# a1q123456/image_stitching

Measured on AMD Instinct MI355X. Metric: 4K frames stitched/sec, higher is better.
Workload: dtype u8

## Files before the change

host/job.cpp:

```cpp
#include "job.hpp"
#include <cstring>

namespace mis {

StitchJob::StitchJob(int device, int width, int height, const std::vector<CameraParams>& cameras, const StitchConfig& cfg)
    : JobCore("mis::StitchJob", "", device, nullptr, width, height, cameras, cfg) {}

StitchJob::~StitchJob() {
    mis_image_free(cctx_, &pano_);
    mis_image_free(cctx_, &mask_);
}

void StitchJob::finalize() {
    if (pano_.data && (pano_.width != key_.pano.width || pano_.height != key_.pano.height)) { mis_image_free(cctx_, &pano_); mis_image_free(cctx_, &mask_); pano_ = MisImage{}; mask_ = MisImage{}; }
    if (!pano_.data) { pano_ = MisImage{}; mask_ = MisImage{}; pano_.mem = mask_.mem = MIS_MEM_DEVICE; }
    check(cctx_, mis_blender_blend(blender_, &pano_, &mask_), "mis_blender_blend");
}

JobOutput StitchJob::run(const std::vector<MisImage>& frames) {
    if ((int)frames.size() != n_) throw std::runtime_error("StitchJob::run: one frame per camera");
    JobOutput out;
    check(cctx_, mis_context_wait(cctx_, ctx_), "mis_context_wait");
    const MisImage* work = work_frames(frames);
    prep_.arm([this] { if (spec_ok_) prepare(everyone_); });
    check(ctx_, mis_orb_on_enqueued(orb_, &Hook::fire, &prep_), "mis_orb_on_enqueued");
    std::vector<MisFeatures> feats(n_);
    std::memset(feats.data(), 0, sizeof(MisFeatures) * n_);
    const int rc_f = mis_orb_detect_batch(orb_, work, n_, feats.data());
    mis_orb_on_enqueued(orb_, nullptr, nullptr);
    check(ctx_, rc_f, "mis_orb_detect_batch");
    prep_.finish();
    for (int i = 0; i < n_; i++) { feats[i].img_idx = i; out.num_features.push_back(feats[i].n); }
    const MisMatchParams mp = reset_matches();
    match_.arm([this, &frames] {
        if (!spec_ok_) return;
        fence_knn();
        compose(frames, everyone_, everyone_);
        finalize();
    });
    check(ctx_, mis_match_on_enqueued(ctx_, &Hook::fire, &match_), "mis_match_on_enqueued");
    const int rc = mis_match_all_pairs(ctx_, feats.data(), n_, &mp, pairwise_.data());
    mis_match_on_enqueued(ctx_, nullptr, nullptr);
    for (auto& f : feats) mis_features_free(ctx_, &f);
    check(ctx_, rc, "mis_match_all_pairs");
    match_.finish();
// ... 23 lines not shown
```

image_stitching_amd/_capi.py:

```python
import ctypes as C
import os
import re

_HERE = os.path.dirname(os.path.abspath(__file__))
LIB_PATH = os.path.join(_HERE, "libmistitch.so")
HEADER_PATH = os.path.join(os.path.dirname(_HERE), "include", "mistitch.h")

MIS_OK = 0
MIS_FENCE_TIMEOUT = 1
MEM_HOST, MEM_DEVICE = 0, 1
U8, S16, F32 = 0, 1, 2
INTER_NEAREST, INTER_LINEAR = 0, 1
BORDER_CONSTANT, BORDER_REFLECT = 0, 2
BLEND_NO, BLEND_FEATHER, BLEND_MULTI_BAND = 0, 1, 2
WARP_SPHERICAL, WARP_CYLINDRICAL, WARP_PLANE = 0, 1, 2


class MisPoint(C.Structure):
    _fields_ = [("x", C.c_int), ("y", C.c_int)]


class MisSize(C.Structure):
    _fields_ = [("width", C.c_int), ("height", C.c_int)]

# ... 59 lines not shown
PROTOTYPES = {
    "mis_context_create": (_i, [_i, _vp, _P(_vp)]),
    "mis_stream_create": (_i, [_i, _i, _P(_vp)]),
    "mis_stream_destroy": (_i, [_vp]),
    "mis_context_destroy": (_i, [_vp]),
    "mis_context_synchronize": (_i, [_vp]),
    "mis_context_wait": (_i, [_vp, _vp]),
    "mis_last_error": (C.c_char_p, [_vp]),
    "mis_version": (C.c_char_p, []),
    "mis_image_free": (_i, [_vp, _P(MisImage)]),
    "mis_orb_default_params": (None, [_P(MisOrbParams)]),
    "mis_orb_create": (_i, [_vp, _P(MisOrbParams), _i, _i, _P(_vp)]),
    "mis_orb_destroy": (_i, [_vp]),
    "mis_orb_detect": (_i, [_vp, _P(MisImage), _P(MisFeatures)]),
    "mis_orb_detect_batch": (_i, [_vp, _P(MisImage), _i, _P(MisFeatures)]),
    "mis_orb_on_enqueued": (_i, [_vp, _vp, _vp]),
    "mis_features_download": (_i, [_vp, _P(MisFeatures), _vp, _vp]),
    "mis_features_upload": (_i, [_vp, _i, _i, _i, _vp, _vp, _i, _i, _P(MisFeatures)]),
    "mis_features_free": (_i, [_vp, _P(MisFeatures)]),
    "mis_orb_debug_level": (_i, [_vp, _i, _i, _vp, _P(_i), _P(_i)]),
    "mis_sift_default_params": (None, [_P(MisSiftParams)]),
    "mis_sift_create": (_i, [_vp, _P(MisSiftParams), _i, _i, _P(_vp)]),
    "mis_sift_destroy": (_i, [_vp]),
    "mis_sift_detect": (_i, [_vp, _P(MisImage), _P(MisFeatures)]),
    "mis_sift_detect_batch": (_i, [_vp, _P(MisImage), _i, _P(MisFeatures)]),
    "mis_sift_debug_level": (_i, [_vp, _P(MisImage), _i, _i, _i, _vp, _P(_i), _P(_i)]),
    "mis_match_default_params": (None, [_P(MisMatchParams)]),
    "mis_match_all_pairs": (_i, [_vp, _P(MisFeatures), _i, _P(MisMatchParams), _P(MisMatchesInfo)]),
    "mis_match_pairs_sharded": (_i, [_vp, _P(MisFeatures), _i, _P(MisMatchParams), _i, _i, _P(MisMatchesInfo)]),
    "mis_matches_free": (_i, [_P(MisMatchesInfo), _i]),
# ... 81 lines not shown
```

image_stitching_amd/csrc/common.h:

```cpp
#pragma once
#include <hip/hip_runtime.h>
#include <stdint.h>
#include <stdio.h>
#include <string.h>
#include <string>
#include <vector>
#include "../../include/mistitch.h"

struct MisWorkspace {
    virtual ~MisWorkspace() {}
};

struct MisContext {
    int device = 0;
    int num_cu = 256;
    MisWorkspace* match_ws = nullptr;
    MisWorkspace* resize_ws = nullptr;
    std::vector<std::pair<size_t, void*>> pool;
    hipStream_t stream = nullptr;
    bool own_stream = false;
    std::string err;
    void* stage = nullptr;
    size_t stage_bytes = 0;
    hipStream_t aux[2] = {nullptr, nullptr};
    void* roi_pinned = nullptr;
    size_t roi_pinned_bytes = 0;
    void* host_stage = nullptr;
    size_t host_stage_bytes = 0;
};

int mis_set_error(MisContext* ctx, int code, const char* fmt, ...);
int mis_host_stage(MisContext* ctx, size_t bytes, void** out);
int mis_dev_stage(MisContext* ctx, size_t bytes, void** out);
int mis_pool_alloc(MisContext* ctx, size_t bytes, void** out, size_t* got, MisContext* errs = nullptr);
int mis_aux_stream(MisContext* ctx, int k, hipStream_t* out);
void mis_pool_free(MisContext* ctx, void* p, size_t bytes);
int mis_feat_block_alloc(MisContext* ctx, size_t bytes, void** out, MisContext* errs = nullptr);

#define MIS_HIP(ctx, call)                                                                             \
    do {                                                                                               \
        hipError_t e_ = (call);                                                                        \
// ... 39 lines not shown
```

image_stitching_amd/csrc/context.hip:

```cpp
#include "common.h"
#include <mutex>
#include <stdarg.h>

int mis_set_error(MisContext* ctx, int code, const char* fmt, ...) {
    char buf[512];
    va_list ap;
    va_start(ap, fmt);
    vsnprintf(buf, sizeof(buf), fmt, ap);
    va_end(ap);
    if (ctx) ctx->err = buf;
    return code;
}

static std::mutex g_pool_mutex;
int mis_pool_alloc(MisContext* ctx, size_t bytes, void** out, size_t* got, MisContext* errs) {
    std::lock_guard<std::mutex> lock(g_pool_mutex);
    int best = -1;
    for (int i = 0; i < (int)ctx->pool.size(); i++)
        if (ctx->pool[i].first >= bytes && ctx->pool[i].first <= 2 * bytes && (best < 0 || ctx->pool[i].first < ctx->pool[best].first)) best = i;
    if (best >= 0) {
        *out = ctx->pool[best].second; *got = ctx->pool[best].first;
        ctx->pool.erase(ctx->pool.begin() + best);
        return MIS_OK;
    }
// ... 52 lines not shown
    ctx->stream = (hipStream_t)stream;
    *out = ctx;
    return MIS_OK;
}

extern "C" int mis_context_destroy(MisContext* ctx) {
    if (!ctx) return MIS_OK;
    hipSetDevice(ctx->device);
    hipStreamSynchronize(ctx->stream);
    delete ctx->match_ws;
    delete ctx->resize_ws;
    for (auto& b : ctx->pool) hipFree(b.second);
    if (ctx->stage) hipFree(ctx->stage);
    if (ctx->roi_pinned) hipHostFree(ctx->roi_pinned);
    if (ctx->host_stage) hipHostFree(ctx->host_stage);
    for (hipStream_t& a : ctx->aux) if (a) { hipStreamSynchronize(a); hipStreamDestroy(a); a = nullptr; }
    if (ctx->own_stream) hipStreamDestroy(ctx->stream);
    delete ctx;
    return MIS_OK;
}

extern "C" int mis_stream_create(int device, int priority, void** out) {
    if (!out) return MIS_E_INVALID;
    *out = nullptr;
    if (hipSetDevice(device) != hipSuccess) return MIS_E_HIP;
    int least = 0, greatest = 0;
    if (hipDeviceGetStreamPriorityRange(&least, &greatest) != hipSuccess) return MIS_E_HIP;
    const int pr = priority > 0 ? least : (priority < 0 ? greatest : 0);
    hipStream_t s = nullptr;
    if (hipStreamCreateWithPriority(&s, hipStreamNonBlocking, pr) != hipSuccess) return MIS_E_HIP;
// ... 137 lines not shown
```

image_stitching_amd/csrc/match.hip:

```cpp
#include "common.h"
#include <thread>
#include <chrono>
#include <atomic>
#include "dev_math.h"
#include "homography.h"
#include <algorithm>
#include <vector>

namespace {

struct FeatDev {
    const uint8_t* desc;
    const MisKeyPoint* kps;
    int n, w, h;
};

struct PairDesc {
    int i, j;
    size_t knn_off12, knn_off21;
    size_t m_off;
    int cap;
};

constexpr int KNN_TILE = 256;
// ... 546 lines not shown

void invert3(const double* H, double* I) {
    double d = H[0] * (H[4] * H[8] - H[5] * H[7]) - H[1] * (H[3] * H[8] - H[5] * H[6]) + H[2] * (H[3] * H[7] - H[4] * H[6]);
    if (d != 0.) d = 1. / d;
    I[0] = (H[4] * H[8] - H[5] * H[7]) * d; I[1] = (H[2] * H[7] - H[1] * H[8]) * d; I[2] = (H[1] * H[5] - H[2] * H[4]) * d;
    I[3] = (H[5] * H[6] - H[3] * H[8]) * d; I[4] = (H[0] * H[8] - H[2] * H[6]) * d; I[5] = (H[2] * H[3] - H[0] * H[5]) * d;
    I[6] = (H[3] * H[7] - H[4] * H[6]) * d; I[7] = (H[1] * H[6] - H[0] * H[7]) * d; I[8] = (H[0] * H[4] - H[1] * H[3]) * d;
}

struct Arena {
    void* p = nullptr;
    size_t bytes = 0;
    bool host = false;
    hipError_t reserve(size_t need) {
        if (need <= bytes) return hipSuccess;
        if (p) { hipError_t e = host ? hipHostFree(p) : hipFree(p); p = nullptr; bytes = 0; if (e != hipSuccess) return e; }
        need = need + need / 4 + 4096;
        hipError_t e = host ? hipHostMalloc(&p, need, hipHostMallocDefault) : hipMalloc(&p, need);
        if (e == hipSuccess) bytes = need;
        return e;
    }
    void release() { if (p) { if (host) hipHostFree(p); else hipFree(p); } p = nullptr; bytes = 0; }
};

struct MatchWorkspace : MisWorkspace {
    Arena dev, pinned, l2;
    HomoBatch b1, b2, b3;
    hipStream_t side = nullptr, third = nullptr;
    OwnedEvent ev_phase0, ev_side_done, ev_phase1, ev_third_done, ev_matches;
    OwnedEvent ev_knn;
    OwnedEvent ev_draw1;
    OwnedEvent tev[8];
    hipEvent_t ev_gate = nullptr;
    std::atomic<long long> seq{0}, knn_seq{0};
    OwnedEvent ev_lists;
    void (*enqueued_cb)(void*) = nullptr;
    void* enqueued_user = nullptr;
    MatchWorkspace() { pinned.host = true; }
    ~MatchWorkspace() override {
        dev.release(); pinned.release(); l2.release();
        homo_batch_release(&b1); homo_batch_release(&b2); homo_batch_release(&b3);
    }
    hipError_t events_ready() {
        for (OwnedEvent* e : {&ev_knn, &ev_matches, &ev_lists, &ev_phase0, &ev_draw1, &ev_side_done, &ev_phase1, &ev_third_done})
            if (const hipError_t r = e->ready()) return r;
        return hipSuccess;
    }
};

MatchWorkspace* workspace(MisContext* ctx) {
    if (!ctx->match_ws) ctx->match_ws = new MatchWorkspace();
    return static_cast<MatchWorkspace*>(ctx->match_ws);
}

struct Carver {
    uintptr_t base = 0;
    size_t off = 0;
    size_t take(size_t bytes) { size_t o = off; off += mis_align_up(bytes ? bytes : 1, 256); return o; }
    void* at(size_t bytes) { return (void*)(base + take(bytes)); }
// ... 283 lines not shown
    MIS_HIP(ctx, hipSetDevice(ctx->device));
    const auto t_begin = std::chrono::steady_clock::now();
    struct SeqGuard {
        MatchWorkspace* ws; long long seq;
        ~SeqGuard() { if (ws->knn_seq.load() < seq) ws->knn_seq.store(seq); }
    } seq_guard{workspace(ctx), 0};
    seq_guard.seq = ++seq_guard.ws->seq;
    for (int i = 0; i < n * n; i++) init_info(&out[i]);
    MatchPlan pl;
    int rc;
    if ((rc = plan_match(ctx, feats, n, rank, world, &pl)) != MIS_OK) return rc;
    const int np = (int)pl.pairs.size();
    if (np == 0) return MIS_OK;
    MatchWorkspace* ws = workspace(ctx);
    hipStream_t st = ctx->stream;
    MIS_HIP(ctx, hipStreamSynchronize(st));
    MatchDev d; MatchPinned h;
    if ((rc = carve_dev(ctx, ws->dev, pl, &d)) != MIS_OK) return rc;
    for (HomoBatch* b : {&ws->b1, &ws->b2, &ws->b3})
        if ((rc = homo_batch_reserve(ctx, b, np, (long long)pl.m_total, p->max_iters)) != MIS_OK) return rc;
    if ((rc = carve_pinned(ctx, ws->pinned, pl, &h)) != MIS_OK) return rc;
    memcpy(h.feats, pl.fd.data(), sizeof(FeatDev) * n);
    memcpy(h.pairs, pl.pairs.data(), sizeof(PairDesc) * np);
    MIS_HIP(ctx, hipMemcpyAsync(d.feats, h.feats, sizeof(FeatDev) * n, hipMemcpyHostToDevice, st));
    MIS_HIP(ctx, hipMemcpyAsync(d.pairs, h.pairs, sizeof(PairDesc) * np, hipMemcpyHostToDevice, st));
    *h.l2_bad = 0;
    if ((rc = enqueue_knn(ctx, ws, pl, feats, d, h)) != MIS_OK) return rc;
    MIS_HIP(ctx, ws->events_ready());
    MIS_HIP(ctx, hipEventRecord(ws->ev_knn.ev, st));
    ws->ev_gate = ws->ev_knn.ev;
    hipLaunchKernelGGL(ratio_union_kernel, dim3(np), dim3(1024), 0, st, (const FeatDev*)d.feats, (const PairDesc*)d.pairs, (const int*)d.idx,
                       (const float*)d.dist, 1.f - p->match_conf, d.matches, d.src, d.dst, d.nm);
    hipLaunchKernelGGL(first_calls_kernel, dim3((np + 127) / 128), dim3(128), 0, st, (const PairDesc*)d.pairs, np, (const int*)d.nm, (const float*)d.src,
                       (const float*)d.dst, d.mask, p->num_matches_thresh1, ws->b1.calls, d.out);
    if ((rc = enqueue_chains(ctx, ws, np, p, d, h)) != MIS_OK) {
        if (ws->side) hipStreamSynchronize(ws->side);
        if (ws->third) hipStreamSynchronize(ws->third);
        hipStreamSynchronize(st);
        return rc;
    }
    MIS_HIP(ctx, hipGetLastError());
    enqueue_results(ws, np, pl.m_total, d, h, st);
    ws->knn_seq.store(seq_guard.seq);
    if (ws->enqueued_cb) {
        void (*cb)(void*) = ws->enqueued_cb;
        void* user = ws->enqueued_user;
        ws->enqueued_cb = nullptr; ws->enqueued_user = nullptr;
        cb(user);
        MIS_HIP(ctx, hipSetDevice(ctx->device));
    }
    const auto tq = std::chrono::steady_clock::now();
    std::chrono::steady_clock::time_point ts;
    if ((rc = assemble_matches(ctx, ws, pl, h, n, out, &ts)) != MIS_OK) return rc;
    if (match_trace()) trace_report(ws, t_begin, tq, ts);
    return MIS_OK;
}

// ... 165 lines not shown
```

image_stitching_amd/csrc/orb.hip:

```cpp
#include "common.h"
#include "dev_math.h"
#include <algorithm>
#include <cmath>
#include <mutex>
#include <unordered_map>

#define ORB_MAX_LEVELS 16
#define ORB_BORDER 32

namespace {

struct LevelDesc {
    int w, h;
    int pp;
    int sp;
    size_t pad_off;
    size_t map_off;
    float scale;
    int nfeat;
    int n2;
    int tiles_x, tiles_y, tile_off;
    int cap1, cand_off;
    int cap2, fin_off;
    int tab_off;
// ... 849 lines not shown
#ifndef DD_UNROLL
#define DD_UNROLL 1
#endif
#pragma unroll DD_UNROLL
    for (int bit = 0; bit < 4; bit++) {
        float x0 = (float)pat[4 * bit], y0 = (float)pat[4 * bit + 1], x1 = (float)pat[4 * bit + 2], y1 = (float)pat[4 * bit + 3];
        int ix0 = mis_round_f(x0 * ca - y0 * sa), iy0 = mis_round_f(x0 * sa + y0 * ca);
        int ix1 = mis_round_f(x1 * ca - y1 * sa), iy1 = mis_round_f(x1 * sa + y1 * ca);
        const int t0 = blurred(ix0, iy0), t1 = blurred(ix1, iy1);
        val |= (t0 < t1) << (bit + 4 * h);
    }
    val |= __shfl_xor(val, 32);
    if (h == 0) desc[(size_t)i * 32 + b] = (uint8_t)val;
}

constexpr int ORB_GATHER_MAX = 96;
struct GatherPtrs { const int* p[ORB_GATHER_MAX]; };
__global__ void gather_ints_kernel(GatherPtrs g, int n, int* __restrict__ out) {
    const int i = blockIdx.x * blockDim.x + threadIdx.x;
    if (i < n) out[i] = *g.p[i];
}

}

struct MisOrb {
    MisContext* ctx = nullptr;
    void (*enqueued_cb)(void*) = nullptr;
    void* enqueued_user = nullptr;
    MisOrbParams p;
    int max_w = 0, max_h = 0;
    int cur_w = 0, cur_h = 0;
    Levels L;
    Work w;
    size_t ws_stride = 0;
    int ws_frames = 0;
    int umax_host[64] = {0};
    int8_t pattern_host[1024] = {0};
    void* mem = nullptr;
    size_t pad_bytes = 0, map_bytes = 0;
    int cand_total = 0, fin_total = 0, tab_total = 0, surv_total = 0, out_cap = 0;
    std::vector<int> tab_host;
    int* host_counts = nullptr;
    bool direct_describe = false;
};

namespace {

void linear_exact_coeffs(int dlen, int slen, int* ofs, int* m1) {
    double inv = (double)dlen / (double)slen, scale = 1.0 / inv;
    for (int i = 0; i < dlen; i++) {
        double v = ((double)i + 0.5) * scale - 0.5;
        int iv = (int)floor(v);
        if (iv < 0) { ofs[i] = 0; m1[i] = 0; }
        else if (iv >= slen - 1) { ofs[i] = slen - 1; m1[i] = 0; }
        else { ofs[i] = iv; m1[i] = (int)lrint((v - (double)iv) * 256.0); }
    }
}
// ... 84 lines not shown
    std::lock_guard<std::mutex> lock(g_feat_mutex);
    g_feat_sizes[mem] = got;
    return MIS_OK;
}

inline uint32_t* feat_lxy(const MisFeatures* f, int cap) {
    size_t kb = mis_align_up(sizeof(MisKeyPoint) * (size_t)cap, 256), db = mis_align_up((size_t)cap * f->desc_cols * mis_dtype_size(f->desc_dtype), 256);
    return (uint32_t*)((uint8_t*)f->owner_ + kb + db);
}
inline int* feat_count(const MisFeatures* f, int cap) {
    size_t kb = mis_align_up(sizeof(MisKeyPoint) * (size_t)cap, 256), db = mis_align_up((size_t)cap * f->desc_cols * mis_dtype_size(f->desc_dtype), 256);
    size_t lb = mis_align_up(sizeof(uint32_t) * (size_t)cap, 256);
    return (int*)((uint8_t*)f->owner_ + kb + db + lb);
}

int enqueue_detect_group(MisOrb* o, const DevView* img, int w, int h, MisFeatures* out, int ng) {
    MisContext* ctx = o->ctx;
    const Levels& L = o->L;
    const Work& W = o->w;
    hipStream_t st = ctx->stream;
    const LevelDesc& d0 = L.d[0];
    const size_t ws = o->ws_stride;
    const unsigned nf = (unsigned)ng;
    OrbIO io;
    for (int k = 0; k < ORB_BATCH; k++) {
        const int q = k < ng ? k : 0;
        io.src[k] = (const uint8_t*)img[q].data; io.sstride[k] = img[q].stride;
        io.aligned[k] = (img[q].stride % 4 == 0) && ((uintptr_t)img[q].data % 4 == 0);
        io.kps[k] = out[q].keypoints; io.lxy[k] = feat_lxy(&out[q], o->out_cap); io.n_dev[k] = feat_count(&out[q], o->out_cap);
        io.desc[k] = (uint8_t*)out[q].descriptors;
    }
// ... 6 lines not shown
                           d.h, d.pp, W.tab + d.tab_off, ws);
    }
    const int pw0 = d0.w + 2 * ORB_BORDER, ph0 = d0.h + 2 * ORB_BORDER;
    hipLaunchKernelGGL((border_kernel<true>), dim3((d0.h * 16 + 255) / 256, 1, L.n * nf), dim3(256), 0, st, L, W.pad, ws);
    hipLaunchKernelGGL((border_kernel<false>), dim3((pw0 + 1023) / 1024, 2 * ORB_BORDER / 4, L.n * nf), dim3(256), 0, st, L, W.pad, ws);
    dim3 gmap((d0.w + FT_COLS - 1) / FT_COLS, (d0.h + FT_ROWS - 1) / FT_ROWS, L.n * nf);
    hipLaunchKernelGGL(fast_nms_kernel, gmap, dim3(256), 0, st, L, W.pad, W.hist, W.tile_cnt, W.surv_xy, W.surv_sc, ws);
    hipLaunchKernelGGL(fast_cut_kernel, dim3(L.n, nf), dim3(256), 0, st, L, W.hist, W.thr, W.flags, ws);
    hipLaunchKernelGGL(compact_kernel, dim3((d0.tiles_x * d0.tiles_y + CT_TILES - 1) / CT_TILES, L.n, nf), dim3(256), 0, st, L, W.tile_cnt, W.surv_xy, W.surv_sc, W.thr, W.cnt1,
                       W.cand_xy, W.cand_resp, ws);
    const int use_harris = o->p.score_type == 0;
    if (use_harris)
        hipLaunchKernelGGL(harris_kernel, dim3((L.d[0].cap1 + 255) / 256, L.n, nf), dim3(256), 0, st, L, W.pad, W.cnt1, W.cand_xy, W.cand_resp, ws);
    hipLaunchKernelGGL(select_rank_kernel, dim3(L.n, nf), dim3(1024), 0, st, L, W.cnt1, W.cand_xy, W.cand_resp, W.cnt2, W.fin_xy, W.fin_resp, W.flags,
                       use_harris, ws);
    hipLaunchKernelGGL(assemble_angle_kernel, dim3((o->out_cap + 3) / 4, nf), dim3(256), 0, st, L, W.pad, W.cnt2, W.fin_xy, W.fin_resp, W.umax, io, o->out_cap, ws, o->direct_describe ? 0 : 1);
    if (o->direct_describe) {
        UMax16 um16;
        for (int v = 0; v < 16; v++) um16.v[v] = o->umax_host[v];
        hipLaunchKernelGGL(describe_direct_kernel, dim3((o->out_cap + 3) / 4, nf), dim3(256), 0, st, L, W.pad, io, W.pattern, W.umax, um16, ws);
    } else {
        for (int k = 0; k < ng; k++) {
            hipLaunchKernelGGL(blur_kernel, dim3((pw0 + 63) / 64, (ph0 + 31) / 32, L.n), dim3(256), 0, st, L, W.pad + k * ws, W.blur + k * ws);
            hipLaunchKernelGGL(describe_kernel, dim3((o->out_cap + 7) / 8), dim3(256), 0, st, L, W.blur + k * ws, out[k].keypoints, io.lxy[k], io.n_dev[k], W.pattern,
                               (uint8_t*)out[k].descriptors);
        }
    }
    MIS_HIP(ctx, hipGetLastError());
    return MIS_OK;
}
// ... 43 lines not shown
    W.tab = (int*)(m + o_tab); W.umax = (int*)(m + o_umax); W.pattern = (int8_t*)(m + o_pat);
    return MIS_OK;
}

int orb_init_workspace(MisOrb* o) {
    MisContext* ctx = o->ctx;
    const Work& W = o->w;
    MIS_HIP(ctx, hipMemcpyAsync(W.umax, o->umax_host, sizeof(o->umax_host), hipMemcpyHostToDevice, ctx->stream));
    MIS_HIP(ctx, hipMemcpyAsync(W.pattern, o->pattern_host, sizeof(o->pattern_host), hipMemcpyHostToDevice, ctx->stream));
    MIS_HIP(ctx, hipMemset2DAsync(W.flags, o->ws_stride, 0, 256, (size_t)o->ws_frames, ctx->stream));
    MIS_HIP(ctx, hipStreamSynchronize(ctx->stream));
    return upload_tables(o);
}

int orb_ensure_frames(MisOrb* o, int frames) {
    frames = std::min(frames, ORB_BATCH);
    if (o->ws_frames >= frames) return MIS_OK;
    MisContext* ctx = o->ctx;
    MIS_HIP(ctx, hipStreamSynchronize(ctx->stream));
    void* old = o->mem;
    const Work oldw = o->w;
    const size_t olds = o->ws_stride;
    const int oldf = o->ws_frames;
    int rc = MIS_E_NOMEM;
    for (int f = frames; f > oldf; f = std::max(oldf, f / 2)) {
        if ((rc = orb_alloc_workspace(o, f)) == MIS_OK) break;
    }
    if (rc != MIS_OK) {
        o->mem = old; o->w = oldw; o->ws_stride = olds; o->ws_frames = oldf;
        return oldf >= 1 ? MIS_OK : rc;
    }
// ... 74 lines not shown
    *out = o;
    return MIS_OK;
}

extern "C" int mis_orb_destroy(MisOrb* o) {
    if (!o) return MIS_OK;
    hipSetDevice(o->ctx->device);
    hipStreamSynchronize(o->ctx->stream);
    if (o->mem) hipFree(o->mem);
    if (o->host_counts) hipHostFree(o->host_counts);
    delete o;
    return MIS_OK;
}


extern "C" int mis_orb_detect_batch(MisOrb* o, const MisImage* imgs, int n, MisFeatures* out) {
    if (!o) return MIS_E_INVALID;
    MisContext* ctx = o->ctx;
    MIS_CHECK(ctx, imgs && out && n >= 1, MIS_E_INVALID, "null argument");
    MIS_HIP(ctx, hipSetDevice(ctx->device));
    int rc;
    for (int i = 0; i < n; i++) {
        if ((rc = check_image(o, &imgs[i])) != MIS_OK) return rc;
        MIS_CHECK(ctx, imgs[i].width == imgs[0].width && imgs[i].height == imgs[0].height, MIS_E_INVALID, "batch frames must share one size");
    }
    if ((rc = replan_if_needed(o, imgs[0].width, imgs[0].height)) != MIS_OK) return rc;
    if ((rc = orb_ensure_frames(o, n)) != MIS_OK) return rc;
    std::vector<DevView> dimg(n);
    for (int i = 0; i < n; i++) memset(&out[i], 0, sizeof(MisFeatures));
    auto fail = [&](int code) {
        hipStreamSynchronize(ctx->stream);
        for (int i = 0; i < n; i++)
            if (out[i].keypoints || out[i].descriptors) mis_features_free(ctx, &out[i]);
        return code;
    };
    for (int i = 0; i < n; i++) {
        out[i].img_idx = i; out[i].img_w = imgs[i].width; out[i].img_h = imgs[i].height;
        if ((rc = alloc_features(ctx, o->out_cap, 32, MIS_U8, &out[i])) != MIS_OK) return fail(rc);
        if ((rc = dimg[i].read(ctx, &imgs[i])) != MIS_OK) return fail(rc);
    }
    const bool trace = getenv("MIS_ORB_TRACE") != nullptr;
    const auto t_enq0 = std::chrono::steady_clock::now();
    for (int g0 = 0; g0 < n; g0 += o->ws_frames) {
        const int ng = std::min(o->ws_frames, n - g0);
        if ((rc = enqueue_detect_group(o, &dimg[g0], imgs[0].width, imgs[0].height, &out[g0], ng)) != MIS_OK) return fail(rc);
    }
    if (trace) fprintf(stderr, "orb batch: %d frames enqueued in %.0f us\n", n, (double)std::chrono::duration_cast<std::chrono::microseconds>(std::chrono::steady_clock::now() - t_enq0).count());
    if (o->enqueued_cb) {
        void (*cb)(void*) = o->enqueued_cb;
        void* user = o->enqueued_user;
        o->enqueued_cb = nullptr; o->enqueued_user = nullptr;
        cb(user);
        MIS_HIP(ctx, hipSetDevice(ctx->device));
    }
    std::vector<int> counts(n);
    const int nl = o->ws_frames;
    std::vector<int> ws_flags(nl, 0);
    if (!o->host_counts) MIS_HIP(ctx, hipHostMalloc((void**)&o->host_counts, sizeof(int) * ORB_GATHER_MAX, hipHostMallocMapped));
    for (int i0 = 0; i0 < n + nl; i0 += ORB_GATHER_MAX) {
        const int m = std::min(ORB_GATHER_MAX, n + nl - i0);
        GatherPtrs gp;
        for (int k = 0; k < m; k++)
            gp.p[k] = i0 + k < n ? feat_count(&out[i0 + k], o->out_cap) : (const int*)((const char*)o->w.flags + (size_t)(i0 + k - n) * o->ws_stride);
        int* dev_view = nullptr;
        MIS_HIP(ctx, hipHostGetDevicePointer((void**)&dev_view, o->host_counts, 0));
        hipLaunchKernelGGL(gather_ints_kernel, dim3(1), dim3(ORB_GATHER_MAX), 0, ctx->stream, gp, m, dev_view);
        MIS_HIP(ctx, hipStreamSynchronize(ctx->stream));
        for (int k = 0; k < m; k++) (i0 + k < n ? counts[i0 + k] : ws_flags[i0 + k - n]) = o->host_counts[k];
    }
    int flags = 0;
    for (int k = 0; k < nl; k++) flags |= ws_flags[k];
    if (flags) hipMemset2DAsync(o->w.flags, o->ws_stride, 0, sizeof(int), (size_t)nl, ctx->stream);
    for (int i = 0; i < n; i++) out[i].n = counts[i];
    if (flags) {
        return mis_set_error(ctx, MIS_E_OVERFLOW, "ORB candidate buffers overflowed (flags %d): too many tied scores", flags);
    }
    return MIS_OK;
}

extern "C" int mis_orb_detect(MisOrb* o, const MisImage* bgr, MisFeatures* out) { return mis_orb_detect_batch(o, bgr, 1, out); }

extern "C" int mis_orb_on_enqueued(MisOrb* o, void (*fn)(void*), void* user) {
    if (!o) return MIS_E_INVALID;
    o->enqueued_cb = fn; o->enqueued_user = user;
    return MIS_OK;
}

extern "C" int mis_features_download(MisContext* ctx, const MisFeatures* f, MisKeyPoint* kps, void* desc) {
    if (!ctx || !f) return MIS_E_INVALID;
    MIS_HIP(ctx, hipSetDevice(ctx->device));
    if (f->n > 0) {
        if (kps) MIS_HIP(ctx, hipMemcpyAsync(kps, f->keypoints, sizeof(MisKeyPoint) * (size_t)f->n, hipMemcpyDeviceToHost, ctx->stream));
        if (desc) MIS_HIP(ctx, hipMemcpyAsync(desc, f->descriptors, (size_t)f->n * f->desc_cols * mis_dtype_size(f->desc_dtype), hipMemcpyDeviceToHost, ctx->stream));
    }
    MIS_HIP(ctx, hipStreamSynchronize(ctx->stream));
// ... 9 lines not shown
    memset(out, 0, sizeof(*out));
    out->img_w = img_w; out->img_h = img_h;
    int rc = alloc_features(ctx, std::max(n, 1), desc_cols, desc_dtype, out);
    if (rc != MIS_OK) return rc;
    if (n) {
        MIS_HIP(ctx, hipMemcpyAsync(out->keypoints, kps, sizeof(MisKeyPoint) * (size_t)n, hipMemcpyHostToDevice, ctx->stream));
        MIS_HIP(ctx, hipMemcpyAsync(out->descriptors, desc, (size_t)n * desc_cols * mis_dtype_size(desc_dtype), hipMemcpyHostToDevice, ctx->stream));
        MIS_HIP(ctx, hipStreamSynchronize(ctx->stream));
    }
    out->n = n;
    return MIS_OK;
}

extern "C" int mis_features_free(MisContext* ctx, MisFeatures* f) {
    if (!ctx || !f) return MIS_E_INVALID;
    if (f->owner_) {
        size_t bytes = 0;
        {
            std::lock_guard<std::mutex> lock(g_feat_mutex);
            auto it = g_feat_sizes.find(f->owner_);
            if (it != g_feat_sizes.end()) { bytes = it->second; g_feat_sizes.erase(it); }
        }
        if (bytes) mis_pool_free(ctx, f->owner_, bytes);
        else {
            MIS_HIP(ctx, hipSetDevice(ctx->device));
            MIS_HIP(ctx, hipStreamSynchronize(ctx->stream));
            MIS_HIP(ctx, hipFree(f->owner_));
        }
    }
    f->owner_ = nullptr; f->keypoints = nullptr; f->descriptors = nullptr; f->n = 0;
// ... 42 lines not shown
```

image_stitching_amd/distributed.py:

```python
import ctypes as C
import os
import time

import numpy as np
import torch

from . import _capi as capi
from . import stitching as st


def frame_block(n, rank, world):
    base, rem = divmod(n, world)
    lo = rank * base + min(rank, rem)
    return list(range(lo, lo + base + (1 if rank < rem else 0)))


class Comm:

    def __init__(self, rank=0, world=1, group=None, always_collective=False):
        self.rank, self.world, self.group = rank, world, group
        self._stage = False
        self._solo = world == 1 and not always_collective
        if not self._solo:
            import torch.distributed as dist
# ... 98 lines not shown
        self.compose_stream = torch.cuda.ExternalStream(h.value, device=ctx.device)
        self.cctx = st.Context(ctx.device.index, stream=h.value)
        self.exchange_device = ctx.device
        self.speculative_compose = True

    def work_frames(self, frames):
        if self.work_scale == 1.0 or not frames:
            return frames
        while len(self._work_frames) < len(frames):
            self._work_frames.append(st._empty_image(self.ctx, self.work_size[1], self.work_size[0], 3, torch.uint8))
        return st.resize_batch(self.ctx, frames, self.work_scale, self.work_scale, out=self._work_frames[:len(frames)])

    def detect(self, frames):
        return self.finder.detect_batch(self.work_frames(frames))

    def feature_counts(self, feats):
        return torch.tensor([len(f) for f in feats], dtype=torch.int32, device=self.ctx.device)

    def pack_features(self, feats, cap):
        m = len(feats)
        dev = self.ctx.device
        rb = self._row_bytes(feats)
        kps = torch.empty((m, cap * 24), dtype=torch.uint8, device=dev)
        desc = torch.empty((m, cap * rb), dtype=torch.uint8, device=dev)
        if m:
            arr = (capi.MisFeatures * m)()
            for k, f in enumerate(feats):
                C.memmove(C.byref(arr[k]), C.byref(f.raw), C.sizeof(capi.MisFeatures))
            self.ctx.check(self.ctx.lib.mis_features_pack(self.ctx.h, arr, m, int(cap), int(rb), C.c_void_p(kps.data_ptr()), C.c_void_p(desc.data_ptr())))
        return kps, desc
# ... 227 lines not shown
        self.cams0 = cameras
        self.work_cams0 = cameras if self.work_scale == 1.0 else [st.scaled_camera(c, self.work_scale) for c in cameras]
        self.cams = self.work_cams0
        self.n = len(cameras)
        self.rank, self.world = rank, world_size
        self.comm = Comm(rank, world_size, group, always_collective)
        self.my_frames = frame_block(self.n, rank, world_size)
        self.frame_size = frame_size
        self.scale = st.Stitcher.warped_image_scale(self.cams)
        self.force_collectives = force_collectives
        self.seam_needed = self.cfg.expos_comp_type != "no" or self.cfg.seam_find_type != "no"
        counts = {len(frame_block(self.n, r, world_size)) for r in range(world_size)}
        if len(counts) != 1:
            raise ValueError("the frame count must divide evenly over the ranks")

    def stage_features(self, frames):
        return self.engine.detect([frames[i] for i in self.my_frames])

    def stage_gather(self, local_feats):
        if self.world == 1 and not self.force_collectives:
            return local_feats
        counts_all = self.comm.all_gather(self.engine.feature_counts(local_feats)).flatten(0, 1)
        cap = max(int(counts_all.max()), 1)
        kps, desc = self.engine.pack_features(local_feats, cap)
        kps_all = self.comm.all_gather(kps).flatten(0, 1)
        desc_all = self.comm.all_gather(desc).flatten(0, 1)
        return self.engine.unpack_features(kps_all, desc_all, counts_all)

    def stage_match(self, feats):
        pm = self.engine.match(feats, self.rank, self.world)
        if self.world == 1 and not self.force_collectives and isinstance(self.engine, HipEngine):
            return pm, self.engine.confidence_tensor(pm, self.n, on_device=False)
# ... 202 lines not shown
            finder = getattr(self.engine, "finder", None)
            box0 = {}

            def prep():
                try:
                    with torch.cuda.stream(self.engine.compose_stream):
                        box0["p"] = self.stage_compose_prepare(list(range(self.n)))
                except BaseException as e:
                    box0["e"] = e
            hooked = hasattr(finder, "on_enqueued") and len(self.my_frames) > 0
            if hooked:
                finder.on_enqueued(prep)
            else:
                prep()
            try:
                local = self.stage_features(frames)
            finally:
                if hooked:
                    finder.on_enqueued(None)
            if "p" not in box0 and "e" not in box0:
                prep()
            if "e" in box0:
                raise box0["e"]
            prepared = box0["p"]
            feats = self.stage_gather(local)
        else:
            feats = self.stage_gather(self.stage_features(frames))
        mark("features")
        if spec:
            import threading
            everyone = list(range(self.n))
            box = {}

            fence = self.engine.match_fence_target() if hasattr(self.engine, "match_fence_target") else None

            solo = self.world == 1 and not self.force_collectives

            def work():
                try:
                    if fence is not None:
                        self.engine.compose_after_knn(fence)
                    mark("compose: fence passed")
# ... 82 lines not shown
```

image_stitching_amd/stitching.py:

```python
import ctypes as C
import math
from dataclasses import dataclass, field

import numpy as np

from . import _capi as capi

try:
    import torch
except Exception:
    torch = None


class MisError(RuntimeError):
    def __init__(self, code, text):
        super().__init__("libmistitch error %d: %s" % (code, text))
        self.code = code


KP_DTYPE = np.dtype([("x", "f4"), ("y", "f4"), ("size", "f4"), ("angle", "f4"), ("response", "f4"), ("octave", "i4")])
DMATCH_DTYPE = np.dtype([("query_idx", "i4"), ("train_idx", "i4"), ("img_idx", "i4"), ("distance", "f4")])

_TORCH_DT = {}
if torch is not None:
# ... 552 lines not shown
    def on_enqueued(self, fn):
        if fn is None:
            self._enqueued_fn = None
            self.ctx.lib.mis_orb_on_enqueued(self.h, None, None)
            return
        self._enqueued_fn = fn
        if getattr(self, "_enqueued_cb", None) is None:
            self._enqueued_cb = C.CFUNCTYPE(None, C.c_void_p)(self._run_enqueued)
        self.ctx.check(self.ctx.lib.mis_orb_on_enqueued(self.h, C.cast(self._enqueued_cb, C.c_void_p), None))

    def _run_enqueued(self, _user):
        fn, self._enqueued_fn = getattr(self, "_enqueued_fn", None), None
        if fn is not None:
            fn()

    def detect_batch(self, imgs):
        n = len(imgs)
        arr = (capi.MisImage * n)(*[as_image(i) for i in imgs])
        raws = (capi.MisFeatures * n)()
        self.ctx.check(self.ctx.lib.mis_orb_detect_batch(self.h, arr, n, raws))
        out = []
        for k in range(n):
            r = capi.MisFeatures()
            C.memmove(C.byref(r), C.byref(raws[k]), C.sizeof(capi.MisFeatures))
            r.img_idx = k
            out.append(ImageFeatures(self.ctx, r))
        return out

    def debug_level(self, level, which):
        w, h = C.c_int(), C.c_int()
        self.ctx.check(self.ctx.lib.mis_orb_debug_level(self.h, level, which, None, C.byref(w), C.byref(h)))
        out = np.zeros((h.value, w.value), np.uint8)
        self.ctx.check(self.ctx.lib.mis_orb_debug_level(self.h, level, which, out.ctypes.data_as(C.c_void_p), C.byref(w), C.byref(h)))
        return out

    def close(self):
        if getattr(self, "h", None) and self.ctx.h:
            self.ctx.lib.mis_orb_destroy(self.h)
        self.h = None

    def __del__(self):
        try:
# ... 476 lines not shown
```

include/mistitch.h:

```cpp
#ifndef MISTITCH_H
#define MISTITCH_H

#include <stddef.h>
#include <stdint.h>

#ifdef __cplusplus
extern "C" {
#endif

#define MIS_OK 0
#define MIS_E_INVALID (-1)
#define MIS_E_HIP (-2)
#define MIS_E_NOMEM (-3)
#define MIS_E_OVERFLOW (-4)
#define MIS_E_STATE (-5)
#define MIS_E_UNSUPPORTED (-6)
#define MIS_FENCE_TIMEOUT 1

enum { MIS_MEM_HOST = 0, MIS_MEM_DEVICE = 1 };
enum { MIS_U8 = 0, MIS_S16 = 1, MIS_F32 = 2 };
enum { MIS_INTER_NEAREST = 0, MIS_INTER_LINEAR = 1 };
enum { MIS_BORDER_CONSTANT = 0, MIS_BORDER_REFLECT = 2 };
enum { MIS_WARP_SPHERICAL = 0, MIS_WARP_CYLINDRICAL = 1, MIS_WARP_PLANE = 2 };
enum { MIS_BLEND_NO = 0, MIS_BLEND_FEATHER = 1, MIS_BLEND_MULTI_BAND = 2 };
// ... 38 lines not shown
typedef struct {
    int img_idx;
    int img_w, img_h;
    int n;
    MisKeyPoint* keypoints;
    void* descriptors;
    int desc_cols, desc_dtype;
    void* owner_;
} MisFeatures;

void mis_orb_default_params(MisOrbParams* p);
int mis_orb_create(MisContext* ctx, const MisOrbParams* p, int max_width, int max_height, MisOrb** out);
int mis_orb_destroy(MisOrb* orb);
int mis_orb_detect(MisOrb* orb, const MisImage* bgr, MisFeatures* out);
int mis_orb_detect_batch(MisOrb* orb, const MisImage* bgr, int n_images, MisFeatures* out);
int mis_orb_on_enqueued(MisOrb* orb, void (*fn)(void*), void* user);
int mis_features_download(MisContext* ctx, const MisFeatures* f, MisKeyPoint* kps_host, void* desc_host);
int mis_features_upload(MisContext* ctx, int img_w, int img_h, int n, const MisKeyPoint* kps_host,
                        const void* desc_host, int desc_cols, int desc_dtype, MisFeatures* out);
int mis_features_free(MisContext* ctx, MisFeatures* f);
int mis_features_pack(MisContext* ctx, const MisFeatures* feats, int m, int cap, int row_bytes, void* kps_dst, void* desc_dst);
int mis_copy_2d(MisContext* ctx, void* dst, size_t dst_pitch, const void* src, size_t src_pitch, size_t width_bytes, size_t height);
int mis_orb_debug_level(MisOrb* orb, int level, int which, uint8_t* host_out, int* width, int* height);

typedef struct {
    float match_conf;
    int num_matches_thresh1, num_matches_thresh2;
    double ransac_thresh;
    int max_iters;
    double confidence;
} MisMatchParams;

typedef struct { int query_idx, train_idx, img_idx; float distance; } MisDMatch;

typedef struct {
    int src_img_idx, dst_img_idx;
    int n_matches;
    MisDMatch* matches;
// ... 109 lines not shown
```

Baseline: 3387.

## Make ORB detection asynchronous and publish counts mid-pipeline via mapped memory

Adds an async ORB batch entry point that writes per-frame keypoint counts and overflow flags to mapped host memory from a small kernel right after rank selection. The host waits on an event recorded at that point instead of synchronizing the whole stream after descriptor computation, so matching can be enqueued while descriptors are still being built. Matching replaces its blanket stream synchronize with event-based waits. The new reserve path adds a device-wide synchronize before frees, and cross-module event bookkeeping brings some ordering risk.

```diff
diff --git a/host/job.cpp b/host/job.cpp
--- a/host/job.cpp
+++ b/host/job.cpp
@@ -26,9 +26,9 @@
     check(ctx_, mis_orb_on_enqueued(orb_, &Hook::fire, &prep_), "mis_orb_on_enqueued");
     std::vector<MisFeatures> feats(n_);
     std::memset(feats.data(), 0, sizeof(MisFeatures) * n_);
-    const int rc_f = mis_orb_detect_batch(orb_, work, n_, feats.data());
+    const int rc_f = mis_orb_detect_batch_async(orb_, work, n_, feats.data());
     mis_orb_on_enqueued(orb_, nullptr, nullptr);
-    check(ctx_, rc_f, "mis_orb_detect_batch");
+    check(ctx_, rc_f, "mis_orb_detect_batch_async");
     prep_.finish();
     for (int i = 0; i < n_; i++) { feats[i].img_idx = i; out.num_features.push_back(feats[i].n); }
     const MisMatchParams mp = reset_matches();
diff --git a/image_stitching_amd/_capi.py b/image_stitching_amd/_capi.py
--- a/image_stitching_amd/_capi.py
+++ b/image_stitching_amd/_capi.py
@@ -97,6 +97,9 @@
     "mis_orb_destroy": (_i, [_vp]),
     "mis_orb_detect": (_i, [_vp, _P(MisImage), _P(MisFeatures)]),
     "mis_orb_detect_batch": (_i, [_vp, _P(MisImage), _i, _P(MisFeatures)]),
+    "mis_orb_detect_batch_async": (_i, [_vp, _P(MisImage), _i, _P(MisFeatures)]),
+    "mis_orb_detect_wait": (_i, [_vp]),
+    "mis_orb_debug_workspaces": (_i, [_vp, _i]),
     "mis_orb_on_enqueued": (_i, [_vp, _vp, _vp]),
     "mis_features_download": (_i, [_vp, _P(MisFeatures), _vp, _vp]),
     "mis_features_upload": (_i, [_vp, _i, _i, _i, _vp, _vp, _i, _i, _P(MisFeatures)]),
diff --git a/image_stitching_amd/csrc/common.h b/image_stitching_amd/csrc/common.h
--- a/image_stitching_amd/csrc/common.h
+++ b/image_stitching_amd/csrc/common.h
@@ -25,6 +25,8 @@
     hipStream_t aux[2] = {nullptr, nullptr};
     void* roi_pinned = nullptr;
     size_t roi_pinned_bytes = 0;
+    hipEvent_t feat_done = nullptr;
+    bool feat_pending = false;
     void* host_stage = nullptr;
     size_t host_stage_bytes = 0;
 };
diff --git a/image_stitching_amd/csrc/context.hip b/image_stitching_amd/csrc/context.hip
--- a/image_stitching_amd/csrc/context.hip
+++ b/image_stitching_amd/csrc/context.hip
@@ -90,6 +90,7 @@
     if (ctx->stage) hipFree(ctx->stage);
     if (ctx->roi_pinned) hipHostFree(ctx->roi_pinned);
     if (ctx->host_stage) hipHostFree(ctx->host_stage);
+    if (ctx->feat_done) hipEventDestroy(ctx->feat_done);
     for (hipStream_t& a : ctx->aux) if (a) { hipStreamSynchronize(a); hipStreamDestroy(a); a = nullptr; }
     if (ctx->own_stream) hipStreamDestroy(ctx->stream);
     delete ctx;
diff --git a/image_stitching_amd/csrc/match.hip b/image_stitching_amd/csrc/match.hip
--- a/image_stitching_amd/csrc/match.hip
+++ b/image_stitching_amd/csrc/match.hip
@@ -584,7 +584,7 @@
     bool host = false;
     hipError_t reserve(size_t need) {
         if (need <= bytes) return hipSuccess;
-        if (p) { hipError_t e = host ? hipHostFree(p) : hipFree(p); p = nullptr; bytes = 0; if (e != hipSuccess) return e; }
+        if (p) { hipError_t e = hipDeviceSynchronize(); if (e == hipSuccess) e = host ? hipHostFree(p) : hipFree(p); p = nullptr; bytes = 0; if (e != hipSuccess) return e; }
         need = need + need / 4 + 4096;
         hipError_t e = host ? hipHostMalloc(&p, need, hipHostMallocDefault) : hipMalloc(&p, need);
         if (e == hipSuccess) bytes = need;
@@ -604,6 +604,8 @@
     hipEvent_t ev_gate = nullptr;
     std::atomic<long long> seq{0}, knn_seq{0};
     OwnedEvent ev_lists;
+    OwnedEvent ev_results;
+    bool results_recorded = false, unfinished = false;
     void (*enqueued_cb)(void*) = nullptr;
     void* enqueued_user = nullptr;
     MatchWorkspace() { pinned.host = true; }
@@ -612,7 +614,7 @@
         homo_batch_release(&b1); homo_batch_release(&b2); homo_batch_release(&b3);
     }
     hipError_t events_ready() {
-        for (OwnedEvent* e : {&ev_knn, &ev_matches, &ev_lists, &ev_phase0, &ev_draw1, &ev_side_done, &ev_phase1, &ev_third_done})
+        for (OwnedEvent* e : {&ev_results, &ev_knn, &ev_matches, &ev_lists, &ev_phase0, &ev_draw1, &ev_side_done, &ev_phase1, &ev_third_done})
             if (const hipError_t r = e->ready()) return r;
         return hipSuccess;
     }
@@ -926,7 +928,10 @@
     if (np == 0) return MIS_OK;
     MatchWorkspace* ws = workspace(ctx);
     hipStream_t st = ctx->stream;
-    MIS_HIP(ctx, hipStreamSynchronize(st));
+    MIS_HIP(ctx, ws->events_ready());
+    if (ws->unfinished) { MIS_HIP(ctx, hipStreamSynchronize(st)); ws->unfinished = false; }
+    else if (ws->results_recorded) MIS_HIP(ctx, hipEventSynchronize(ws->ev_results.ev));
+    ws->unfinished = true;
     MatchDev d; MatchPinned h;
     if ((rc = carve_dev(ctx, ws->dev, pl, &d)) != MIS_OK) return rc;
     for (HomoBatch* b : {&ws->b1, &ws->b2, &ws->b3})
@@ -938,7 +943,6 @@
     MIS_HIP(ctx, hipMemcpyAsync(d.pairs, h.pairs, sizeof(PairDesc) * np, hipMemcpyHostToDevice, st));
     *h.l2_bad = 0;
     if ((rc = enqueue_knn(ctx, ws, pl, feats, d, h)) != MIS_OK) return rc;
-    MIS_HIP(ctx, ws->events_ready());
     MIS_HIP(ctx, hipEventRecord(ws->ev_knn.ev, st));
     ws->ev_gate = ws->ev_knn.ev;
     hipLaunchKernelGGL(ratio_union_kernel, dim3(np), dim3(1024), 0, st, (const FeatDev*)d.feats, (const PairDesc*)d.pairs, (const int*)d.idx,
@@ -953,6 +957,8 @@
     }
     MIS_HIP(ctx, hipGetLastError());
     enqueue_results(ws, np, pl.m_total, d, h, st);
+    MIS_HIP(ctx, hipEventRecord(ws->ev_results.ev, st));
+    ws->results_recorded = true; ws->unfinished = false;
     ws->knn_seq.store(seq_guard.seq);
     if (ws->enqueued_cb) {
         void (*cb)(void*) = ws->enqueued_cb;
diff --git a/image_stitching_amd/csrc/orb.hip b/image_stitching_amd/csrc/orb.hip
--- a/image_stitching_amd/csrc/orb.hip
+++ b/image_stitching_amd/csrc/orb.hip
@@ -887,11 +887,15 @@
     if (h == 0) desc[(size_t)i * 32 + b] = (uint8_t)val;
 }
 
-constexpr int ORB_GATHER_MAX = 96;
-struct GatherPtrs { const int* p[ORB_GATHER_MAX]; };
-__global__ void gather_ints_kernel(GatherPtrs g, int n, int* __restrict__ out) {
-    const int i = blockIdx.x * blockDim.x + threadIdx.x;
-    if (i < n) out[i] = *g.p[i];
+__global__ __launch_bounds__(64) void publish_counts_kernel(int nlevels, const int* cnt2, const int* flags, int cap_out, size_t ws, int ng,
+                                                            int* __restrict__ counts_out, int* __restrict__ flags_out) {
+    const int fr = threadIdx.x;
+    if (fr >= ng) return;
+    WS_OFF(cnt2, fr, ws); WS_OFF(flags, fr, ws);
+    int total = 0;
+    for (int l = 0; l < nlevels; l++) total += cnt2[l];
+    counts_out[fr] = min(total, cap_out);
+    flags_out[fr] = flags[0];
 }
 
 }
@@ -907,6 +911,7 @@
     Work w;
     size_t ws_stride = 0;
     int ws_frames = 0;
+    int ws_limit = ORB_BATCH;
     int umax_host[64] = {0};
     int8_t pattern_host[1024] = {0};
     void* mem = nullptr;
@@ -914,6 +919,9 @@
     int cand_total = 0, fin_total = 0, tab_total = 0, surv_total = 0, out_cap = 0;
     std::vector<int> tab_host;
     int* host_counts = nullptr;
+    int* host_counts_dev = nullptr;
+    int host_cap = 0;
+    OwnedEvent ev_counts;
     bool direct_describe = false;
 };
 
@@ -1028,7 +1036,7 @@
     return (int*)((uint8_t*)f->owner_ + kb + db + lb);
 }
 
-int enqueue_detect_group(MisOrb* o, const DevView* img, int w, int h, MisFeatures* out, int ng) {
+int enqueue_detect_group(MisOrb* o, const DevView* img, int w, int h, MisFeatures* out, int ng, int* counts_dev, int* flags_dev, hipEvent_t ev_counts) {
     MisContext* ctx = o->ctx;
     const Levels& L = o->L;
     const Work& W = o->w;
@@ -1065,6 +1073,8 @@
         hipLaunchKernelGGL(harris_kernel, dim3((L.d[0].cap1 + 255) / 256, L.n, nf), dim3(256), 0, st, L, W.pad, W.cnt1, W.cand_xy, W.cand_resp, ws);
     hipLaunchKernelGGL(select_rank_kernel, dim3(L.n, nf), dim3(1024), 0, st, L, W.cnt1, W.cand_xy, W.cand_resp, W.cnt2, W.fin_xy, W.fin_resp, W.flags,
                        use_harris, ws);
+    hipLaunchKernelGGL(publish_counts_kernel, dim3(1), dim3(64), 0, st, L.n, W.cnt2, W.flags, o->out_cap, ws, ng, counts_dev, flags_dev);
+    if (ev_counts) MIS_HIP(ctx, hipEventRecord(ev_counts, st));
     hipLaunchKernelGGL(assemble_angle_kernel, dim3((o->out_cap + 3) / 4, nf), dim3(256), 0, st, L, W.pad, W.cnt2, W.fin_xy, W.fin_resp, W.umax, io, o->out_cap, ws, o->direct_describe ? 0 : 1);
     if (o->direct_describe) {
         UMax16 um16;
@@ -1138,7 +1148,7 @@
 }
 
 int orb_ensure_frames(MisOrb* o, int frames) {
-    frames = std::min(frames, ORB_BATCH);
+    frames = std::min(frames, o->ws_limit);
     if (o->ws_frames >= frames) return MIS_OK;
     MisContext* ctx = o->ctx;
     MIS_HIP(ctx, hipStreamSynchronize(ctx->stream));
@@ -1243,7 +1253,17 @@
 }
 
 
-extern "C" int mis_orb_detect_batch(MisOrb* o, const MisImage* imgs, int n, MisFeatures* out) {
+extern "C" int mis_orb_detect_wait(MisOrb* o) {
+    if (!o) return MIS_E_INVALID;
+    MisContext* ctx = o->ctx;
+    if (!ctx->feat_pending) return MIS_OK;
+    MIS_HIP(ctx, hipSetDevice(ctx->device));
+    MIS_HIP(ctx, hipEventSynchronize(ctx->feat_done));
+    ctx->feat_pending = false;
+    return MIS_OK;
+}
+
+extern "C" int mis_orb_detect_batch_async(MisOrb* o, const MisImage* imgs, int n, MisFeatures* out) {
     if (!o) return MIS_E_INVALID;
     MisContext* ctx = o->ctx;
     MIS_CHECK(ctx, imgs && out && n >= 1, MIS_E_INVALID, "null argument");
@@ -1255,10 +1275,23 @@
     }
     if ((rc = replan_if_needed(o, imgs[0].width, imgs[0].height)) != MIS_OK) return rc;
     if ((rc = orb_ensure_frames(o, n)) != MIS_OK) return rc;
-    std::vector<DevView> dimg(n);
+    MIS_HIP(ctx, o->ev_counts.ready());
+    if (!ctx->feat_done) MIS_HIP(ctx, hipEventCreateWithFlags(&ctx->feat_done, hipEventDisableTiming));
+    const int nl = o->ws_frames, ngroups = (n + nl - 1) / nl, need = n + ngroups * nl;
+    if (o->host_cap < need) {
+        MIS_HIP(ctx, hipStreamSynchronize(ctx->stream));
+        if (o->host_counts) { MIS_HIP(ctx, hipHostFree(o->host_counts)); o->host_counts = nullptr; o->host_counts_dev = nullptr; o->host_cap = 0; }
+        MIS_HIP(ctx, hipHostMalloc((void**)&o->host_counts, sizeof(int) * (size_t)(need + 64), hipHostMallocMapped));
+        MIS_HIP(ctx, hipHostGetDevicePointer((void**)&o->host_counts_dev, o->host_counts, 0));
+        o->host_cap = need + 64;
+    }
+    DevView few[ORB_BATCH];
+    std::vector<DevView> many(n > ORB_BATCH ? n : 0);
+    DevView* dimg = n > ORB_BATCH ? many.data() : few;
     for (int i = 0; i < n; i++) memset(&out[i], 0, sizeof(MisFeatures));
     auto fail = [&](int code) {
         hipStreamSynchronize(ctx->stream);
+        ctx->feat_pending = false;
         for (int i = 0; i < n; i++)
             if (out[i].keypoints || out[i].descriptors) mis_features_free(ctx, &out[i]);
         return code;
@@ -1268,46 +1301,58 @@
         if ((rc = alloc_features(ctx, o->out_cap, 32, MIS_U8, &out[i])) != MIS_OK) return fail(rc);
         if ((rc = dimg[i].read(ctx, &imgs[i])) != MIS_OK) return fail(rc);
     }
-    const bool trace = getenv("MIS_ORB_TRACE") != nullptr;
+    static const bool trace = getenv("MIS_ORB_TRACE") != nullptr;
     const auto t_enq0 = std::chrono::steady_clock::now();
-    for (int g0 = 0; g0 < n; g0 += o->ws_frames) {
-        const int ng = std::min(o->ws_frames, n - g0);
-        if ((rc = enqueue_detect_group(o, &dimg[g0], imgs[0].width, imgs[0].height, &out[g0], ng)) != MIS_OK) return fail(rc);
-    }
-    if (trace) fprintf(stderr, "orb batch: %d frames enqueued in %.0f us\n", n, (double)std::chrono::duration_cast<std::chrono::microseconds>(std::chrono::steady_clock::now() - t_enq0).count());
+    auto us_since = [&]() { return (double)std::chrono::duration_cast<std::chrono::microseconds>(std::chrono::steady_clock::now() - t_enq0).count(); };
+    for (int g0 = 0, g = 0; g0 < n; g0 += nl, g++) {
+        const int ng = std::min(nl, n - g0);
+        const bool last = g0 + nl >= n;
+        if ((rc = enqueue_detect_group(o, &dimg[g0], imgs[0].width, imgs[0].height, &out[g0], ng, o->host_counts_dev + g0, o->host_counts_dev + n + g * nl,
+                                       last ? o->ev_counts.ev : nullptr)) != MIS_OK)
+            return fail(rc);
+    }
+    if (hipEventRecord(ctx->feat_done, ctx->stream) != hipSuccess) return fail(mis_set_error(ctx, MIS_E_HIP, "hipEventRecord failed (%s:%d)", __FILE__, __LINE__));
+    ctx->feat_pending = true;
+    if (trace) fprintf(stderr, "orb batch: %d frames enqueued in %.0f us\n", n, us_since());
     if (o->enqueued_cb) {
         void (*cb)(void*) = o->enqueued_cb;
         void* user = o->enqueued_user;
         o->enqueued_cb = nullptr; o->enqueued_user = nullptr;
         cb(user);
-        MIS_HIP(ctx, hipSetDevice(ctx->device));
-    }
-    std::vector<int> counts(n);
-    const int nl = o->ws_frames;
-    std::vector<int> ws_flags(nl, 0);
-    if (!o->host_counts) MIS_HIP(ctx, hipHostMalloc((void**)&o->host_counts, sizeof(int) * ORB_GATHER_MAX, hipHostMallocMapped));
-    for (int i0 = 0; i0 < n + nl; i0 += ORB_GATHER_MAX) {
-        const int m = std::min(ORB_GATHER_MAX, n + nl - i0);
-        GatherPtrs gp;
-        for (int k = 0; k < m; k++)
-            gp.p[k] = i0 + k < n ? feat_count(&out[i0 + k], o->out_cap) : (const int*)((const char*)o->w.flags + (size_t)(i0 + k - n) * o->ws_stride);
-        int* dev_view = nullptr;
-        MIS_HIP(ctx, hipHostGetDevicePointer((void**)&dev_view, o->host_counts, 0));
-        hipLaunchKernelGGL(gather_ints_kernel, dim3(1), dim3(ORB_GATHER_MAX), 0, ctx->stream, gp, m, dev_view);
-        MIS_HIP(ctx, hipStreamSynchronize(ctx->stream));
-        for (int k = 0; k < m; k++) (i0 + k < n ? counts[i0 + k] : ws_flags[i0 + k - n]) = o->host_counts[k];
-    }
+        if (hipSetDevice(ctx->device) != hipSuccess) return fail(mis_set_error(ctx, MIS_E_HIP, "hipSetDevice failed (%s:%d)", __FILE__, __LINE__));
+    }
+    {
+        const hipError_t e = hipEventSynchronize(o->ev_counts.ev);
+        if (e != hipSuccess) return fail(mis_set_error(ctx, MIS_E_HIP, "hipEventSynchronize failed: %s (%s:%d)", hipGetErrorString(e), __FILE__, __LINE__));
+    }
+    if (trace) fprintf(stderr, "orb batch: counts known %.0f us after the first enqueue\n", us_since());
+    const volatile int* hc = o->host_counts;
     int flags = 0;
-    for (int k = 0; k < nl; k++) flags |= ws_flags[k];
-    if (flags) hipMemset2DAsync(o->w.flags, o->ws_stride, 0, sizeof(int), (size_t)nl, ctx->stream);
-    for (int i = 0; i < n; i++) out[i].n = counts[i];
+    for (int g0 = 0, g = 0; g0 < n; g0 += nl, g++)
+        for (int k = 0; k < std::min(nl, n - g0); k++) flags |= hc[n + g * nl + k];
     if (flags) {
+        hipMemset2DAsync(o->w.flags, o->ws_stride, 0, sizeof(int), (size_t)nl, ctx->stream);
+        fail(MIS_E_OVERFLOW);
         return mis_set_error(ctx, MIS_E_OVERFLOW, "ORB candidate buffers overflowed (flags %d): too many tied scores", flags);
     }
-    return MIS_OK;
+    for (int i = 0; i < n; i++) out[i].n = hc[i];
+    return MIS_OK;
+}
+
+extern "C" int mis_orb_detect_batch(MisOrb* o, const MisImage* imgs, int n, MisFeatures* out) {
+    const int rc = mis_orb_detect_batch_async(o, imgs, n, out);
+    if (rc != MIS_OK) return rc;
+    return mis_orb_detect_wait(o);
 }
 
 extern "C" int mis_orb_detect(MisOrb* o, const MisImage* bgr, MisFeatures* out) { return mis_orb_detect_batch(o, bgr, 1, out); }
+
+extern "C" int mis_orb_debug_workspaces(MisOrb* o, int max_frames) {
+    if (!o) return MIS_E_INVALID;
+    MIS_CHECK(o->ctx, max_frames >= 1, MIS_E_INVALID, "at least one workspace");
+    o->ws_limit = std::min(max_frames, ORB_BATCH);
+    return MIS_OK;
+}
 
 extern "C" int mis_orb_on_enqueued(MisOrb* o, void (*fn)(void*), void* user) {
     if (!o) return MIS_E_INVALID;
@@ -1347,6 +1392,11 @@
 
 extern "C" int mis_features_free(MisContext* ctx, MisFeatures* f) {
     if (!ctx || !f) return MIS_E_INVALID;
+    if (f->owner_ && ctx->feat_pending) {
+        MIS_HIP(ctx, hipSetDevice(ctx->device));
+        if (hipEventQuery(ctx->feat_done) != hipSuccess) MIS_HIP(ctx, hipEventSynchronize(ctx->feat_done));
+        ctx->feat_pending = false;
+    }
     if (f->owner_) {
         size_t bytes = 0;
         {
diff --git a/image_stitching_amd/distributed.py b/image_stitching_amd/distributed.py
--- a/image_stitching_amd/distributed.py
+++ b/image_stitching_amd/distributed.py
@@ -136,6 +136,11 @@
     def detect(self, frames):
         return self.finder.detect_batch(self.work_frames(frames))
 
+    def detect_async(self, frames):
+        if isinstance(self.finder, st.OrbFeatureFinder):
+            return self.finder.detect_batch(self.work_frames(frames), wait=False)
+        return self.detect(frames)
+
     def feature_counts(self, feats):
         return torch.tensor([len(f) for f in feats], dtype=torch.int32, device=self.ctx.device)
 
@@ -393,8 +398,11 @@
         if len(counts) != 1:
             raise ValueError("the frame count must divide evenly over the ranks")
 
-    def stage_features(self, frames):
-        return self.engine.detect([frames[i] for i in self.my_frames])
+    def stage_features(self, frames, then_match=False):
+        mine = [frames[i] for i in self.my_frames]
+        if then_match and self.world == 1 and not self.force_collectives and hasattr(self.engine, "detect_async"):
+            return self.engine.detect_async(mine)
+        return self.engine.detect(mine)
 
     def stage_gather(self, local_feats):
         if self.world == 1 and not self.force_collectives:
@@ -627,7 +635,7 @@
             else:
                 prep()
             try:
-                local = self.stage_features(frames)
+                local = self.stage_features(frames, then_match=True)
             finally:
                 if hooked:
                     finder.on_enqueued(None)
@@ -638,7 +646,7 @@
             prepared = box0["p"]
             feats = self.stage_gather(local)
         else:
-            feats = self.stage_gather(self.stage_features(frames))
+            feats = self.stage_gather(self.stage_features(frames, then_match=True))
         mark("features")
         if spec:
             import threading
diff --git a/image_stitching_amd/stitching.py b/image_stitching_amd/stitching.py
--- a/image_stitching_amd/stitching.py
+++ b/image_stitching_amd/stitching.py
@@ -590,11 +590,12 @@
         if fn is not None:
             fn()
 
-    def detect_batch(self, imgs):
+    def detect_batch(self, imgs, wait=True):
         n = len(imgs)
         arr = (capi.MisImage * n)(*[as_image(i) for i in imgs])
         raws = (capi.MisFeatures * n)()
-        self.ctx.check(self.ctx.lib.mis_orb_detect_batch(self.h, arr, n, raws))
+        entry = self.ctx.lib.mis_orb_detect_batch if wait else self.ctx.lib.mis_orb_detect_batch_async
+        self.ctx.check(entry(self.h, arr, n, raws))
         out = []
         for k in range(n):
             r = capi.MisFeatures()
@@ -602,6 +603,9 @@
             r.img_idx = k
             out.append(ImageFeatures(self.ctx, r))
         return out
+
+    def wait(self):
+        self.ctx.check(self.ctx.lib.mis_orb_detect_wait(self.h))
 
     def debug_level(self, level, which):
         w, h = C.c_int(), C.c_int()
diff --git a/include/mistitch.h b/include/mistitch.h
--- a/include/mistitch.h
+++ b/include/mistitch.h
@@ -76,6 +76,8 @@
 int mis_orb_destroy(MisOrb* orb);
 int mis_orb_detect(MisOrb* orb, const MisImage* bgr, MisFeatures* out);
 int mis_orb_detect_batch(MisOrb* orb, const MisImage* bgr, int n_images, MisFeatures* out);
+int mis_orb_detect_batch_async(MisOrb* orb, const MisImage* bgr, int n_images, MisFeatures* out);
+int mis_orb_detect_wait(MisOrb* orb);
 int mis_orb_on_enqueued(MisOrb* orb, void (*fn)(void*), void* user);
 int mis_features_download(MisContext* ctx, const MisFeatures* f, MisKeyPoint* kps_host, void* desc_host);
 int mis_features_upload(MisContext* ctx, int img_w, int img_h, int n, const MisKeyPoint* kps_host,
@@ -84,6 +86,7 @@
 int mis_features_pack(MisContext* ctx, const MisFeatures* feats, int m, int cap, int row_bytes, void* kps_dst, void* desc_dst);
 int mis_copy_2d(MisContext* ctx, void* dst, size_t dst_pitch, const void* src, size_t src_pitch, size_t width_bytes, size_t height);
 int mis_orb_debug_level(MisOrb* orb, int level, int which, uint8_t* host_out, int* width, int* height);
+int mis_orb_debug_workspaces(MisOrb* orb, int max_frames);
 
 typedef struct {
     float match_conf;
```

Measured after the change: 3415 (median of 4 runs). Within noise of the previous version (+0.8%).
